# marcopesavento/Super-resolution-3D-Human-Shape-from-a-Single-Low-Resolution-Image

Hardware: AMD Instinct MI355X
Metric: occupancy queries/sec (dense 512^3 reconstruction: encoder + query sweep + 2x marching cubes) (higher is better)
Workload: dtype bf16

## Files before the change

### super-resolution-3d-human-shape-from-a-single-low-resolution-image_amd/csrc/surs_api.cpp

```cpp
#include "surs_common.h"

extern "C" int surs_abi_version(void) { return SURS_ABI_VERSION; }

extern "C" const char *surs_last_error(void) { return surs::err_buf(); }

extern "C" int surs_device_info(int *cu_count, char *arch_out) {
    int dev = 0;
    SURS_HIP_CHECK(hipGetDevice(&dev));
    hipDeviceProp_t prop;
    SURS_HIP_CHECK(hipGetDeviceProperties(&prop, dev));
    if (cu_count) *cu_count = prop.multiProcessorCount;
    if (arch_out) {
        strncpy(arch_out, prop.gcnArchName, 31);
        arch_out[31] = 0;
    }
    return 0;
}

#include <atomic>
#include <cstdlib>
#include <mutex>

namespace {
struct OptionRow {
    const char *name, *env;
    int def;
    char env_first;
    int env_value;
    const char *what;
};
const OptionRow kOptions[surs::OPT_COUNT] = {
    {"split_parts", "SURS_SPLIT", 2, 'b', 3, "operand parts of the fp32-grade GEMMs: 2 (f16 x 2) or 3 (bf16 x 3; env: bf16x3)"},
    {"grid_f32_columns", "SURS_GRID_F32", 1, 'g', 0, "0 (env: gemm): the fp32 sweep on the per-point layer kernels"},
    {"grid_kernel", "SURS_GRID_KERNEL", 0, 0, 0, "reduced-precision column kernel: 0 (default 12), 3, 10, 12"},
    {"grid_f32_kernel", "SURS_GRID_F32_KERNEL", 0, 0, 0, "fp32-grade column kernel: 0 (default 11), 5, 11"},
    {"r_parts", "SURS_R_PARTS", 1, 0, 0, "1: the bf16 sweep's R vectors from one f16 part; 0: the sweep's split"},
    {"grid_f32_passes", "SURS_GRID_F32_PASSES", 2, 0, 0, "passes of the fp32-grade column kernel per batch: 2 (lr, then hr) or 1"},
    {"bicubic_block", "SURS_BICUBIC_BLOCK", 1, 0, 0, "0: bicubic x2 with statistics one output per item (A/B; same bits)"},
    {"mc_emit_reclassify", "SURS_MC_EMIT_RECLASSIFY", 0, 0, 0, "1: marching cubes' emit pass classifies again (tests)"},
    {"point_runs_speculate", "SURS_POINT_RUNS_SPECULATE", 1, 0, 0, "0: surs_query_points_columns reads the run count before it launches"},
    {"conv_trace", "SURS_CONV_TRACE", 0, 0, 0, "diagnostic builds (-DSURS_CONV_TRACE): print the 3x3 kernel's phase stamps"},
    {"v3_trace", "SURS_V3_TRACE", 0, 0, 0, "diagnostic builds (-DSURS_V3_TRACE): print the column kernels' stamps"},
    {"conv_tall_min_wg", "SURS_CONV_TALL_MIN_WG", 256, 0, 0, "workgroups from which a stride-1 3x3 convolution takes the 8-row tile instead of 4 rows (0: never; same bits)"},
    {"conv_wide_min_wg", "SURS_CONV_WIDE_MIN_WG", 512, 0, 0, "workgroups (of 64 channels) from which such a launch takes 8 rows x 64 channels (part of the bits: another order of sums; 0: never)"},
    {"mc_ring", "SURS_MC_RING", 258, 0, 0, "planes of marching cubes' edge -> vertex-id ring = layers per chunk of a one-piece extraction + 1 (66: round 5's)"},
    {"rvec_small", "SURS_RVEC_SMALL", 1, 0, 0, "0: the affine part's GEMM of batches of <= 1024 columns on the 256 x 256-tile kernel (A/B; same bits)"},
};
std::atomic<int> g_option[surs::OPT_COUNT];
std::once_flag g_option_once;
void import_environment() {
    for (int i = 0; i < surs::OPT_COUNT; ++i) {
        const OptionRow &r = kOptions[i];
        int v = r.def;
        if (const char *e = getenv(r.env)) {
            if (r.env_first) v = (e[0] == r.env_first) ? r.env_value : r.def;
            else if (e[0]) v = atoi(e);
        }
        g_option[i].store(v, std::memory_order_relaxed);
    }
}
int find_option(const char *name) {
    if (!name) return -1;
    for (int i = 0; i < surs::OPT_COUNT; ++i)
        if (!strcmp(name, kOptions[i].name) || !strcmp(name, kOptions[i].env)) return i;
    return -1;
}
}

int surs::option(surs::Opt id) {
    std::call_once(g_option_once, import_environment);
    return g_option[id].load(std::memory_order_relaxed);
}

extern "C" int surs_set_option(const char *name, int value) {
    const int i = find_option(name);
    SURS_REQUIRE(i >= 0, "unknown option '%s' (surs_option_name(i) lists them)", name ? name : "(null)");
    std::call_once(g_option_once, import_environment);
    g_option[i].store(value, std::memory_order_relaxed);
    return 0;
}

extern "C" int surs_get_option(const char *name, int *value) {
    const int i = find_option(name);
    SURS_REQUIRE(i >= 0 && value, "unknown option '%s'", name ? name : "(null)");
    *value = surs::option((surs::Opt)i);
    return 0;
}

extern "C" const char *surs_option_name(int index) { return (index >= 0 && index < surs::OPT_COUNT) ? kOptions[index].name : nullptr; }
extern "C" const char *surs_option_help(int index) { return (index >= 0 && index < surs::OPT_COUNT) ? kOptions[index].what : nullptr; }
```

### super-resolution-3d-human-shape-from-a-single-low-resolution-image_amd/csrc/surs_common.h

```cpp
#pragma once
#include <hip/hip_runtime.h>

#include <cstdarg>
#include <cstdio>
#include <cstring>

#include "../../include/surs.h"

namespace surs {

inline char *err_buf() {
    static thread_local char buf[512] = "";
    return buf;
}

inline int fail(int code, const char *fmt, ...) {
    va_list ap;
    va_start(ap, fmt);
    vsnprintf(err_buf(), 512, fmt, ap);
    va_end(ap);
    return code;
}

#define SURS_HIP_CHECK(expr)                                                                     \
    do {                                                                                         \
        hipError_t e_ = (expr);                                                                  \
        if (e_ != hipSuccess)                                                                    \
            return surs::fail(SURS_E_HIP, "%s:%d %s -> %s", __FILE__, __LINE__, #expr, hipGetErrorString(e_)); \
    } while (0)

#define SURS_LAUNCH_CHECK() SURS_HIP_CHECK(hipGetLastError())

#define SURS_REQUIRE(cond, ...)                                   \
    do {                                                          \
        if (!(cond)) return surs::fail(SURS_E_INVALID, __VA_ARGS__); \
    } while (0)

#ifndef SURS_ABL_NO_ISA_PINS
#define SURS_ISA_PIN(v) asm volatile("" : "+v"(v))
#else
#define SURS_ISA_PIN(v) do { } while (0)
#endif

enum Opt {
    OPT_SPLIT_PARTS, OPT_GRID_F32_COLUMNS, OPT_GRID_KERNEL, OPT_GRID_F32_KERNEL, OPT_R_PARTS,
    OPT_GRID_F32_PASSES, OPT_BICUBIC_BLOCK, OPT_MC_EMIT_RECLASSIFY, OPT_POINT_RUNS_SPECULATE, OPT_CONV_TRACE,
    OPT_V3_TRACE, OPT_CONV_TALL_MIN_WG, OPT_CONV_WIDE_MIN_WG, OPT_MC_RING, OPT_RVEC_SMALL, OPT_COUNT
};
int option(Opt id);

inline hipStream_t as_stream(void *s) { return reinterpret_cast<hipStream_t>(s); }

constexpr int ceil_div(long long a, long long b) { return (int)((a + b - 1) / b); }

struct DeviceOnce {
    unsigned long long mask = 0;
    bool first() {
        int dev = 0;
        if (hipGetDevice(&dev) != hipSuccess || dev < 0 || dev >= 64) return true;
        const unsigned long long bit = 1ull << dev;
        const unsigned long long old = __atomic_fetch_or(&mask, bit, __ATOMIC_ACQ_REL);
        return !(old & bit);
    }
};
inline size_t align_up(size_t v, size_t a) { return (v + a - 1) / a * a; }

}
```

### super-resolution-3d-human-shape-from-a-single-low-resolution-image_amd/csrc/surs_gemm.inc

```
__device__ __forceinline__ bool gemm_block_tile(int mblocks, int nblocks, int &mb, int &nb) {
    const unsigned total = (unsigned)mblocks * (unsigned)nblocks, per = gridDim.x >> 3;
    const unsigned logical = (blockIdx.x & 7u) * per + (blockIdx.x >> 3);
    mb = (int)(logical % (unsigned)mblocks);
    nb = (int)(logical / (unsigned)mblocks);
    return logical < total;
}

static inline unsigned gemm_grid(int mblocks, long long nblocks) {
    const long long total = (long long)mblocks * nblocks;
    return (unsigned)(((total + 7) / 8) * 8);
}

struct SplitSeg {
    const unsigned short *base;
    long long part;
    int ktiles;
};

constexpr int G3_STAGES = 3;
constexpr int g3_stage_bytes(int bm, int np_ = 3) { return np_ * ((bm / 32) + 8) * 1024; }
constexpr int g3_lds_bytes(int bm, int np_ = 3) { return G3_STAGES * g3_stage_bytes(bm, np_); }

template <int NP> struct SplitKind;
template <> struct SplitKind<1> {
// ... 163 lines not shown
        for (int kt = 0; kt < ktiles; ++kt) {
            step_barrier(kt);
            phase1(kt);
            phase2(kt);
        }
    } else {
        step_barrier(0);
        phase1(0);
        for (int kt = 1; kt < ktiles; ++kt) {
            step_barrier(kt);
            phase2(kt - 1);
            phase1(kt);
        }
        phase2(ktiles - 1);
    }

#undef G3_RD
#undef G3_WAIT4
#undef G3_WAIT2
#pragma unroll
    for (int i = 0; i < TI; ++i)
#pragma unroll
        for (int j = 0; j < 2; ++j) {
            const long long n = n0 + wn * 64 + j * 32 + li;
            const int mrow = m0 + wm * (TI * 32) + i * 32;
            if constexpr (OUT == G3_F32_T) {
                const long long nb0 = n0 + wn * 64 + j * 32 + 4 * kh;
                const float bm = bias[mrow + li];
#pragma unroll
                for (int g = 0; g < 4; ++g)
#pragma unroll
                    for (int r = 0; r < 4; ++r) Y[(nb0 + 8 * g + r) * ldy + mrow + li] = acc[i][j][4 * g + r] + bm;
                continue;
            }
            float v[16];
#pragma unroll
            for (int g = 0; g < 4; ++g)
#pragma unroll
                for (int r = 0; r < 4; ++r) {
                    float t = acc[i][j][4 * g + r] + bias[mrow + 8 * g + 4 * kh + r];
                    v[4 * g + r] = t > 0.0f ? t : 0.01f * t;
                }
            if constexpr (OUT == G3_F32) {
#pragma unroll
                for (int g = 0; g < 4; ++g)
#pragma unroll
                    for (int r = 0; r < 4; ++r) Y[(long long)(mrow + 8 * g + 4 * kh + r) * ldy + n] = v[4 * g + r];
            } else
#pragma unroll
            for (int q = 0; q < 2; ++q) {
                unsigned e[NP][2], o[NP][2];
#pragma unroll
                for (int d = 0; d < 2; ++d) {
                    unsigned short x0[NP], x1[NP], y0[NP], y1[NP];
                    SK::split(v[8 * q + 2 * d], x0);
                    SK::split(v[8 * q + 2 * d + 1], x1);
                    SK::split(v[8 * q + 4 + 2 * d], y0);
                    SK::split(v[8 * q + 4 + 2 * d + 1], y1);
#pragma unroll
                    for (int p = 0; p < NP; ++p) {
                        e[p][d] = (unsigned)x0[p] | ((unsigned)x1[p] << 16);
                        o[p][d] = (unsigned)y0[p] | ((unsigned)y1[p] << 16);
                    }
                }
                unsigned short *dst = Ys + ((long long)((mrow >> 4) + q) * np + n) * 16 + kh * 8;
#pragma unroll
                for (int p = 0; p < NP; ++p) {
                    const auto t0 = __builtin_amdgcn_permlane32_swap(e[p][0], o[p][0], false, false);
                    const auto t1 = __builtin_amdgcn_permlane32_swap(e[p][1], o[p][1], false, false);
                    u32x4 w = {t0[0], t1[0], t0[1], t1[1]};
                    *reinterpret_cast<u32x4 *>(dst + p * ys_part) = w;
                }
            }
        }
}



struct RvecSmallArgs {
    const unsigned short *w[2];
    const unsigned short *g[2];
    long long g_part[2];
    long long npm[2];
    float *r[2];
    int wgs0;
};
template <int NP>
__global__ __launch_bounds__(256) void rvec_small_kernel(RvecSmallArgs a) {
    typedef SplitKind<NP> SK;
    typedef typename SK::vec8 vec8;
    constexpr int KT = D1 / 16, PF = 4;
    static_assert(KT % PF == 0, "k-steps in rounds of the prefetch depth");
    const int tid = threadIdx.x, lane = tid & 63, wave = tid >> 6, kh = lane >> 5, li = lane & 31;
    const int m = (int)blockIdx.x >= a.wgs0 ? 1 : 0;
    const int wg = m ? (int)blockIdx.x - a.wgs0 : (int)blockIdx.x;
    const long long npm = a.npm[m];
    const long long n0 = (long long)(wg >> 2) * 64;
    const int m0 = (wg & 3) * 128 + wave * 32;
    const size_t w_part = (size_t)D1 * D2;
    const unsigned short *wp = a.w[m] + (size_t)(m0 / 32) * 512 + lane * 8;
    const unsigned short *xp = a.g[m] + ((size_t)n0 + li) * 16 + kh * 8;
    const long long g_part = a.g_part[m];
    f32x16 acc[2];
#pragma unroll
    for (int j = 0; j < 2; ++j)
#pragma unroll
        for (int q = 0; q < 16; ++q) acc[j][q] = 0.0f;
    vec8 wf[PF][NP], xf[PF][2][NP];
    auto fetch = [&](int kt, int s) {
#pragma unroll
        for (int p = 0; p < NP; ++p) {
            wf[s][p] = *reinterpret_cast<const vec8 *>(wp + (size_t)kt * D2 * 16 + p * w_part);
#pragma unroll
            for (int j = 0; j < 2; ++j) xf[s][j][p] = *reinterpret_cast<const vec8 *>(xp + ((size_t)kt * npm + 32 * j) * 16 + p * g_part);
        }
    };
#pragma unroll
    for (int s = 0; s < PF; ++s) fetch(s, s);
    for (int k0 = 0; k0 < KT; k0 += PF) {
#pragma unroll
        for (int s = 0; s < PF; ++s) {
            vec8 w_[NP], x_[2][NP];
#pragma unroll
            for (int p = 0; p < NP; ++p) {
                w_[p] = wf[s][p];
                x_[0][p] = xf[s][0][p];
                x_[1][p] = xf[s][1][p];
            }
            if (k0 + PF + s < KT) fetch(k0 + PF + s, s);
#pragma unroll
            for (int t = 0; t < NP; ++t)
#pragma unroll
                for (int j = 0; j < 2; ++j) acc[j] = SK::mfma(x_[j][t], w_[NP - 1 - t], acc[j]);
            if (NP == 3) {
#pragma unroll
                for (int j = 0; j < 2; ++j) acc[j] = SK::mfma(x_[j][0], w_[1], acc[j]);
#pragma unroll
                for (int j = 0; j < 2; ++j) acc[j] = SK::mfma(x_[j][1], w_[0], acc[j]);
            }
            if (NP >= 2) {
#pragma unroll
                for (int j = 0; j < 2; ++j) acc[j] = SK::mfma(x_[j][0], w_[0], acc[j]);
            }
        }
    }
    float *out = a.r[m];
#pragma unroll
    for (int j = 0; j < 2; ++j)
#pragma unroll
        for (int gq = 0; gq < 4; ++gq)
#pragma unroll
            for (int r = 0; r < 4; ++r) out[(n0 + 32 * j + 4 * kh + 8 * gq + r) * D2 + m0 + li] = acc[j][4 * gq + r] + 0.0f;
}
```

### super-resolution-3d-human-shape-from-a-single-low-resolution-image_amd/csrc/surs_query.hip

```cpp
#include <hip/hip_runtime.h>

#include <cstdlib>
#include <map>
#include <mutex>
#include <type_traits>
#include <utility>
#include <vector>

#include "surs_common.h"
#include "surs_mlp_generic.h"
#include "surs_mlp_layout.h"

namespace surs {

typedef float f32x16 __attribute__((ext_vector_type(16)));
typedef float f32x4 __attribute__((ext_vector_type(4)));
typedef unsigned u32x4 __attribute__((ext_vector_type(4)));
typedef unsigned u32x2 __attribute__((ext_vector_type(2)));
typedef float f32x2 __attribute__((ext_vector_type(2)));

struct PointSource {
    int mode;
    const float *pts;
    const long long *idx;
// ... 190 lines not shown
                                                       float *__restrict__ pred, float *__restrict__ logit,
                                                       float *__restrict__ p_slot, unsigned short *__restrict__ Fs,
                                                       long long fs_part) {
    const long long t = (long long)blockIdx.x * 256 + threadIdx.x;
    if (t >= n) return;
    float acc = w4[D4 + C0PAD];
    for (int k = 0; k < D4; ++k) acc = fmaf(w4[k], Y3[(long long)k * ld + t], acc);
    for (int k = 0; k < C_G + 2; ++k) acc = fmaf(w4[D4 + k], F[(long long)k * ld + t], acc);
    const float p = mask[t] * (1.0f / (1.0f + expf(-acc)));
    pred[t] = p;
    if (logit) logit[t] = acc;
    if (p_slot) p_slot[t] = p;
    if (Fs) {
        unsigned short parts[NP];
        SplitKind<NP>::split(p, parts);
        unsigned short *dst = Fs + ((long long)(C_G / 16) * ld + t) * 16 + 1;
#pragma unroll
        for (int k = 0; k < NP; ++k) dst[k * fs_part] = parts[k];
    }
}

template <int NP>
__global__ __launch_bounds__(256) void patch_plr_kernel(const float *__restrict__ p_lr, long long ld, long long n, float *__restrict__ p_slot,
                                                        unsigned short *__restrict__ Fs, long long fs_part) {
    const long long t = (long long)blockIdx.x * 256 + threadIdx.x;
    if (t >= n) return;
    const float p = p_lr[t];
    p_slot[t] = p;
    if (Fs) {
        unsigned short parts[NP];
        SplitKind<NP>::split(p, parts);
        unsigned short *dst = Fs + ((long long)(C_G / 16) * ld + t) * 16 + 1;
#pragma unroll
        for (int k = 0; k < NP; ++k) dst[k * fs_part] = parts[k];
    }
}

__global__ __launch_bounds__(256) void mean_views_kernel(const float *__restrict__ in, long long view_stride, int nviews,
                                                         long long count, float inv, float *__restrict__ out) {
    const long long t = (long long)blockIdx.x * 256 + threadIdx.x;
    if (t >= count) return;
    float acc = in[t];
    for (int v = 1; v < nviews; ++v) acc += in[(long long)v * view_stride + t];
    out[t] = acc * inv;
}

template <int NP>
__global__ __launch_bounds__(256) void split_rows_kernel(const float *__restrict__ X, long long ld, int ktiles,
                                                         unsigned short *__restrict__ Xs, long long part) {
    const long long n = (long long)blockIdx.x * 256 + threadIdx.x;
    const int kt = blockIdx.y;
    if (n >= ld) return;
#pragma unroll
    for (int half = 0; half < 2; ++half) {
        u16x8_t q[NP];
#pragma unroll
        for (int j = 0; j < 8; ++j) {
            unsigned short parts[NP];
            SplitKind<NP>::split(X[(long long)(16 * kt + 8 * half + j) * ld + n], parts);
#pragma unroll
            for (int k = 0; k < NP; ++k) q[k][j] = parts[k];
        }
        unsigned short *dst = Xs + ((long long)kt * ld + n) * 16 + half * 8;
#pragma unroll
        for (int k = 0; k < NP; ++k) *reinterpret_cast<u16x8_t *>(dst + k * part) = q[k];
    }
}

template <int NP>
__global__ __launch_bounds__(256) void mlp_last_views_kernel(const float *__restrict__ w4, const float *__restrict__ Y3,
                                                             const float *__restrict__ Fm, long long ld, long long n,
                                                             int nviews, const float *__restrict__ mask ,
                                                             float *__restrict__ pred , float *__restrict__ logit,
                                                             float *__restrict__ p_slot ,
                                                             long long f_view_stride,
                                                             unsigned short *__restrict__ Fs ,
                                                             long long fs_part) {
    const long long t = (long long)blockIdx.x * 256 + threadIdx.x;
    if (t >= n) return;
    float acc = w4[D4 + C0PAD];
    for (int k = 0; k < D4; ++k) acc = fmaf(w4[k], Y3[(long long)k * ld + t], acc);
    for (int k = 0; k < C_G + 2; ++k) acc = fmaf(w4[D4 + k], Fm[(long long)k * ld + t], acc);
    const float y = 1.0f / (1.0f + expf(-acc));
    if (logit) logit[t] = acc;
    for (int v = 0; v < nviews; ++v) {
        const float p = mask[(long long)v * ld + t] * y;
        pred[(long long)v * n + t] = p;
        if (p_slot) p_slot[(long long)v * f_view_stride + t] = p;
        if (Fs) {
            unsigned short parts[NP];
            SplitKind<NP>::split(p, parts);
            unsigned short *dst = Fs + (long long)v * NP * fs_part + ((long long)(C_G / 16) * ld + t) * 16 + 1;
#pragma unroll
            for (int k = 0; k < NP; ++k) dst[k * fs_part] = parts[k];
        }
    }
}

struct Fp32Workspace {
    float *F, *Y3, *mask;
    unsigned short *Fs, *Y0s, *Y1s, *Y2s;
    long long np;
};

static size_t fp32_ws_bytes(long long np) {
    return (size_t)np * ((C0PAD + D4 + 1) * sizeof(float) + (size_t)(C0PAD + D1 + D2 + D3) * 6) + 4096;
}

static Fp32Workspace carve_fp32(void *ws, long long np) {
    Fp32Workspace w;
    float *p = (float *)ws;
    w.np = np;
    w.F = p; p += (size_t)C0PAD * np;
    w.Y3 = p; p += (size_t)D4 * np;
    w.mask = p; p += np;
    unsigned short *q = (unsigned short *)p;
    w.Fs = q; q += (size_t)3 * C0PAD * np;
    w.Y0s = q; q += (size_t)3 * D1 * np;
    w.Y1s = q; q += (size_t)3 * D2 * np;
    w.Y2s = q;
    return w;
}

static int g_split_override = 0;
static thread_local int t_split_call = 0;
static int split_parts() {
    const int v = option(OPT_SPLIT_PARTS) == 3 ? 3 : 2;
    return t_split_call > 1 ? t_split_call : (g_split_override ? g_split_override : v);
}

template <int NP, int... More, class F> static void with_parts(int parts, F &&f) {
    if constexpr (sizeof...(More) == 0) f(std::integral_constant<int, NP>());
    else if (parts == NP) f(std::integral_constant<int, NP>());
    else with_parts<More...>(parts, f);
}

static int g3_set_attributes() {
    static DeviceOnce attr;
    if (attr.first()) {
        SURS_HIP_CHECK(hipFuncSetAttribute((const void *)gemm_x3g_kernel<8, 256, G3_SPLIT, 2>, hipFuncAttributeMaxDynamicSharedMemorySize, g3_lds_bytes(256, 2)));
        SURS_HIP_CHECK(hipFuncSetAttribute((const void *)gemm_x3g_kernel<8, 256, G3_F32, 2>, hipFuncAttributeMaxDynamicSharedMemorySize, g3_lds_bytes(256, 2)));
        SURS_HIP_CHECK(hipFuncSetAttribute((const void *)gemm_x3g_kernel<8, 128, G3_F32, 2>, hipFuncAttributeMaxDynamicSharedMemorySize, g3_lds_bytes(128, 2)));
        SURS_HIP_CHECK(hipFuncSetAttribute((const void *)gemm_x3g_kernel<8, 128, G3_F32_T, 2>, hipFuncAttributeMaxDynamicSharedMemorySize, g3_lds_bytes(128, 2)));
        SURS_HIP_CHECK(hipFuncSetAttribute((const void *)gemm_x3g_kernel<8, 256, G3_SPLIT>, hipFuncAttributeMaxDynamicSharedMemorySize, g3_lds_bytes(256)));
        SURS_HIP_CHECK(hipFuncSetAttribute((const void *)gemm_x3g_kernel<8, 256, G3_F32>, hipFuncAttributeMaxDynamicSharedMemorySize, g3_lds_bytes(256)));
        SURS_HIP_CHECK(hipFuncSetAttribute((const void *)gemm_x3g_kernel<8, 128, G3_F32>, hipFuncAttributeMaxDynamicSharedMemorySize, g3_lds_bytes(128)));
        SURS_HIP_CHECK(hipFuncSetAttribute((const void *)gemm_x3g_kernel<8, 128, G3_F32_T>, hipFuncAttributeMaxDynamicSharedMemorySize, g3_lds_bytes(128)));
        SURS_HIP_CHECK(hipFuncSetAttribute((const void *)gemm_x3g_kernel<8, 256, G3_F32_T, 2>, hipFuncAttributeMaxDynamicSharedMemorySize, g3_lds_bytes(256, 2)));
        SURS_HIP_CHECK(hipFuncSetAttribute((const void *)gemm_x3g_kernel<8, 256, G3_F32_T>, hipFuncAttributeMaxDynamicSharedMemorySize, g3_lds_bytes(256)));
        SURS_HIP_CHECK(hipFuncSetAttribute((const void *)gemm_x3g_kernel<8, 256, G3_F32_T, 1>, hipFuncAttributeMaxDynamicSharedMemorySize, g3_lds_bytes(256, 1)));
        SURS_HIP_CHECK(hipFuncSetAttribute((const void *)gemm_x3g_kernel<8, 256, G3_SPLIT, 1>, hipFuncAttributeMaxDynamicSharedMemorySize, g3_lds_bytes(256, 1)));
        SURS_HIP_CHECK(hipFuncSetAttribute((const void *)gemm_x3g_kernel<8, 256, G3_F32, 1>, hipFuncAttributeMaxDynamicSharedMemorySize, g3_lds_bytes(256, 1)));
        SURS_HIP_CHECK(hipFuncSetAttribute((const void *)gemm_x3g_kernel<8, 128, G3_F32, 1>, hipFuncAttributeMaxDynamicSharedMemorySize, g3_lds_bytes(128, 1)));
    }
    return 0;
}

static int launch_layer(hipStream_t st, int parts, int out, const void *W, int M, SplitSeg s1, SplitSeg s2, long long np, long long n,
                        const float *bias, float *Y, unsigned short *Ys) {
    SURS_REQUIRE(parts >= 1 && parts <= 3, "layer kernel: 1, 2 or 3 operand parts");
    SURS_REQUIRE(np % 256 == 0 && n % 256 == 0 && n <= np, "the layer kernel needs 256-point tiles");
    SURS_REQUIRE(M % 256 == 0 || (out != G3_SPLIT && M % 128 == 0), "layer kernel rows: a multiple of 256 (of 128 for an fp32 output)");
    SURS_REQUIRE(M % 256 == 0 || out != G3_F32_T || parts > 1, "no one-part layer kernel for a transposed output of 128-row tiles");
    int rc = g3_set_attributes();
    if (rc) return rc;
    const int K = 16 * (s1.ktiles + s2.ktiles), nb = (int)(n / 256);
    const long long ldy = out == G3_F32_T ? M : np;
    with_parts<1, 2, 3>(parts, [&](auto NP) {
        auto go = [&](auto BM, auto OUT) {
            hipLaunchKernelGGL((gemm_x3g_kernel<8, BM, OUT, NP>), dim3(gemm_grid(M / BM, nb)), dim3(512), g3_lds_bytes(BM, NP), st,
                               (const unsigned short *)W, M, K, s1, s2, np, bias, Y, ldy, Ys, (long long)M * np, nb);
        };
        using C256 = std::integral_constant<int, 256>;
        using C128 = std::integral_constant<int, 128>;
        if (out == G3_SPLIT) go(C256(), std::integral_constant<int, G3_SPLIT>());
        else if (out == G3_F32) {
            if (M % 256 == 0) go(C256(), std::integral_constant<int, G3_F32>());
            else go(C128(), std::integral_constant<int, G3_F32>());
        } else if (M % 256 == 0) go(C256(), std::integral_constant<int, G3_F32_T>());
        else if constexpr (NP > 1) go(C128(), std::integral_constant<int, G3_F32_T>());
    });
    SURS_LAUNCH_CHECK();
    return 0;
}

static int run_points_fp32(hipStream_t st, const PointSource &src, long long n, const float *feat_lr, int hl, int wl,
                           const float *feat_hr, int hh, int wh, const char *blob, const MlpBlobHeader &h,
                           const Fp32Workspace &w, float *pred_hr, float *pred_lr, float *logit_hr, float *logit_lr,
                           int parts = 0, const float *p_lr_in = nullptr, bool lr_only = false) {
    const long long np = w.np;
    if (parts == 0) parts = t_split_call == 1 ? 1 : split_parts();
    const long long fs_part = (long long)C0PAD * np;
    with_parts<1, 2, 3>(parts, [&](auto NP) {
        hipLaunchKernelGGL(gather_kernel<NP>, dim3((unsigned)ceil_div(n, 64)), dim3(256), 0, st, src, n, feat_lr, hl, wl, feat_hr,
                           hh, wh, w.F, np, w.mask, (float *)nullptr, w.Fs, fs_part);
    });
    SURS_LAUNCH_CHECK();
    if (p_lr_in) {
        with_parts<1, 2, 3>(parts, [&](auto NP) {
            hipLaunchKernelGGL(patch_plr_kernel<NP>, dim3((unsigned)ceil_div(n, 256)), dim3(256), 0, st, p_lr_in, np, n,
                               w.F + (size_t)(C_G + 1) * np, w.Fs, fs_part);
        });
        SURS_LAUNCH_CHECK();
    }
    const SplitSeg none = {nullptr, 0, 0}, f = {w.Fs, fs_part, C0PAD / 16}, y0 = {w.Y0s, (long long)D1 * np, D1 / 16},
                   y1 = {w.Y1s, (long long)D2 * np, D2 / 16}, y2 = {w.Y2s, (long long)D3 * np, D3 / 16};
    for (int m = p_lr_in ? 1 : 0; m < (lr_only ? 1 : 2); ++m) {
        auto W = [&](int l) { return (const void *)(blob + (parts <= 2 ? h.wt2[m][l] : h.wt3[m][l])); };
        auto BI = [&](int l) { return (const float *)(blob + h.bias[m][l]); };
        int rc;
        if ((rc = launch_layer(st, parts, G3_SPLIT, W(0), D1, f, none, np, np, BI(0), nullptr, w.Y0s))) return rc;
        if ((rc = launch_layer(st, parts, G3_SPLIT, W(1), D2, y0, none, np, np, BI(1), nullptr, w.Y1s))) return rc;
        if ((rc = launch_layer(st, parts, G3_SPLIT, W(2), D3, y1, f, np, np, BI(2), nullptr, w.Y2s))) return rc;
        if ((rc = launch_layer(st, parts, G3_F32, W(3), D4, y2, f, np, np, BI(3), w.Y3, nullptr))) return rc;
        with_parts<1, 2, 3>(parts, [&](auto NP) {
            hipLaunchKernelGGL(mlp_last_kernel<NP>, dim3((unsigned)ceil_div(n, 256)), dim3(256), 0, st,
                               (const float *)(blob + h.w4[m]), w.Y3, w.F, np, n, w.mask, m == 0 ? pred_lr : pred_hr,
                               m == 0 ? logit_lr : logit_hr, m == 0 ? w.F + (size_t)(C_G + 1) * np : (float *)nullptr,
                               m == 0 ? w.Fs : (unsigned short *)nullptr, fs_part);
        });
        SURS_LAUNCH_CHECK();
    }
    return 0;
}

template <int DT> struct HalfT;
template <> struct HalfT<SURS_BF16> {
    typedef __bf16 elem;
    typedef __bf16 vec8 __attribute__((ext_vector_type(8)));
    typedef __bf16 vec2 __attribute__((ext_vector_type(2)));
    static __device__ __forceinline__ f32x16 mfma(vec8 a, vec8 b, f32x16 c) {
        return __builtin_amdgcn_mfma_f32_32x32x16_bf16(a, b, c, 0, 0, 0);
    }
};
template <> struct HalfT<SURS_F16> {
    typedef _Float16 elem;
    typedef _Float16 vec8 __attribute__((ext_vector_type(8)));
    typedef _Float16 vec2 __attribute__((ext_vector_type(2)));
    static __device__ __forceinline__ f32x16 mfma(vec8 a, vec8 b, f32x16 c) {
        return __builtin_amdgcn_mfma_f32_32x32x16_f16(a, b, c, 0, 0, 0);
    }
};

struct GridArgs {
    const float *cc;
    const float *colmask;
    const float *zvec;
    const char *core;
    const char *corex;
    const char *b1frag;
    const char *w1t;
    const char *w1tx;
    const float *rvec_lr, *rvec_hr;
    long long rld_lr, rld_hr;
    float zmid;
    unsigned *colctr;
    int phase;
    unsigned long long *kstat;
    float b1_inv_scale;
    float *vol_hr, *vol_lr;
    int ncols, rz;
    int zstride;
    const int *kcount;
    const unsigned short *klist;
    const int *colstart;
    const float *zpts;
    unsigned *ovf_count;
    int *ovf_list;
    char *aimg;
    const int *tile_list;
    const unsigned *tile_count;
    double z0, dz;
    float c22, c23;
    float zmul, zdiv;
};

__device__ __forceinline__ float lrelu_max(float x, float y) { return __builtin_elementwise_maximum(x, y); }
__device__ __forceinline__ float lrelu01(float x) { return lrelu_max(x, 0.01f * x); }

__device__ __forceinline__ unsigned opaque(unsigned v) {
    asm volatile("" : "+v"(v));
    return v;
}
__device__ __forceinline__ unsigned fresh_lane() {
    unsigned v;
    asm volatile("v_mbcnt_lo_u32_b32 %0, -1, 0\n\tv_mbcnt_hi_u32_b32 %0, -1, %0" : "=v"(v));
    return v;
}

#include "surs_grid_v3.inc"
#include "surs_grid_v5.inc"
#include "surs_grid_restated.inc"
#include "surs_grid_v10.inc"
#include "surs_grid_v12.inc"
#include "surs_grid_v11.inc"

template <int NP>
__global__ __launch_bounds__(256) void colsum_prepare_kernel(const float *__restrict__ cc, const float *__restrict__ zvec, int ncp,
                                                             float zmid, unsigned short *__restrict__ g_lr, long long part_lr,
                                                             unsigned short *__restrict__ g_hr, long long part_hr) {
    typedef SplitKind<NP> SK;
    __shared__ __attribute__((aligned(16))) unsigned stage[64][20][8];
    const int tid = threadIdx.x, lane = tid & 63, wave = tid >> 6;
    const int col0 = blockIdx.x * 4, col = col0 + wave;
    const int c16 = lane;
    const float *row = cc + (size_t)col * CC_PAD + 16 * c16;
// ... 429 lines not shown
        const float Z = c23 + c22 * zw;
        return Z * zmul / zdiv;
    };
    unsigned nl = 0, nh = 0;
    for (int k0 = 0; k0 < rz; k0 += tile) {
        const float e0 = zf_of(k0), e1 = zf_of(k0 + tile - 1);
        const float zlo = fminf(e0, e1), zhi = fmaxf(e0, e1);
#pragma unroll
        for (int i = 0; i < 4; ++i) {
            {
                const float xm = fmaf(zmid, zl[i], al[i]);
                const float t0 = zl[i] * zlo, t1 = zl[i] * zhi;
                const float mn = al[i] + fminf(t0, t1), mx = al[i] + fmaxf(t0, t1);
                nl += ((xm > 0.0f) ? (mn > 0.0f) : (mx <= 0.0f)) ? 0u : 1u;
            }
            {
                const float xm = fmaf(0.5f, ph[i], fmaf(zmid, zh[i], ah[i]));
                const float t0 = zh[i] * zlo, t1 = zh[i] * zhi;
                const float mn = ah[i] + fminf(t0, t1) + fminf(0.0f, ph[i]), mx = ah[i] + fmaxf(t0, t1) + fmaxf(0.0f, ph[i]);
                nh += ((xm > 0.0f) ? (mn > 0.0f) : (mx <= 0.0f)) ? 0u : 1u;
            }
        }
    }
#pragma unroll
    for (int d = 32; d >= 1; d >>= 1) {
        nl += __shfl_xor(nl, d);
        nh += __shfl_xor(nh, d);
    }
    if ((tid & 63) == 0) {
        atomicAdd(out, (unsigned long long)nl);
        atomicAdd(out + 1, (unsigned long long)nh);
    }
}

static int query_grid_impl(int i0, int i1, int ry, int rz, const double *mat, const float *calib, float zmul,
                           float zdiv, const float *feat_lr, int hl, int wl, const float *feat_hr, int hh, int wh,
                           const void *mlp_blob, int dtype, void *workspace, size_t workspace_bytes, float *vol_hr,
                           float *vol_lr, int kernel_call, void *stream);

extern "C" int surs_query_grid_opt(int i0, int i1, int ry, int rz, const double *mat, const float *calib, float zmul,
                                   float zdiv, const float *feat_lr, int hl, int wl, const float *feat_hr, int hh, int wh,
                                   const void *mlp_blob, int dtype, void *workspace, size_t workspace_bytes, float *vol_hr,
                                   float *vol_lr, const SursGridOptions *opt, void *stream) {
    int kernel = 0, parts = 0;
    if (opt) {
        kernel = opt->kernel;
        parts = opt->operand_parts;
        SURS_REQUIRE(grid_kernel_known(kernel), "SursGridOptions.kernel: 0, 3, 10, 12 (reduced precision), 5, 11 (fp32-grade)");
        SURS_REQUIRE(parts == 0 || parts == 2 || parts == 3, "SursGridOptions.operand_parts: 0, 2 or 3");
    }
    const int saved = t_split_call;
    if (parts) t_split_call = parts;
    const int rc = query_grid_impl(i0, i1, ry, rz, mat, calib, zmul, zdiv, feat_lr, hl, wl, feat_hr, hh, wh, mlp_blob, dtype, workspace,
                                   workspace_bytes, vol_hr, vol_lr, kernel, stream);
    t_split_call = saved;
    return rc;
}

extern "C" int surs_query_grid(int i0, int i1, int ry, int rz, const double *mat, const float *calib, float zmul,
                               float zdiv, const float *feat_lr, int hl, int wl, const float *feat_hr, int hh, int wh,
                               const void *mlp_blob, int dtype, void *workspace, size_t workspace_bytes, float *vol_hr,
                               float *vol_lr, void *stream) {
    return query_grid_impl(i0, i1, ry, rz, mat, calib, zmul, zdiv, feat_lr, hl, wl, feat_hr, hh, wh, mlp_blob, dtype, workspace,
                           workspace_bytes, vol_hr, vol_lr, 0, stream);
}

namespace {
struct ColumnSweep {
    hipStream_t st;
    const char *blob;
    MlpBlobHeader h;
    int dtype;
    int kver, kver32;
    bool restated;
    const float *feat_lr; int hl, wl;
    const float *feat_hr; int hh, wh;
    const double *mat; const float *calib; float zmul, zdiv;
    void *workspace;
    int cus;
    int kmid;
    const int *run_colstart = nullptr;
    const float *run_z = nullptr;
    const int *run_tiles = nullptr;
    const unsigned *run_ntiles = nullptr;
    long long run_ntiles_host = 0;
};
}

static void resolve_column_kernels(int kernel_call, int &kver, int &kver32) {
    const int ve = option(OPT_GRID_KERNEL), ve32 = option(OPT_GRID_F32_KERNEL);
    const int kver_env = (ve == 3 || ve == 10 || ve == 12) ? ve : SURS_DEFAULT_GRID_KERNEL;
    const int kver32_env = (ve32 == 5 || ve32 == 11) ? ve32 : SURS_DEFAULT_GRID_F32_KERNEL;
    const auto is32 = [](int v) { return v == 5 || v == 11; };
    kver = kver_env;
    kver32 = kver32_env;
    if (g_grid_kernel_override) (is32(g_grid_kernel_override) ? kver32 : kver) = g_grid_kernel_override;
    if (kernel_call) (is32(kernel_call) ? kver32 : kver) = kernel_call;
}

static int device_cus() {
    int dev = 0;
    hipDeviceProp_t prop;
    if (hipGetDevice(&dev) == hipSuccess && hipGetDeviceProperties(&prop, dev) == hipSuccess) return prop.multiProcessorCount;
    return 256;
}

static int run_column_batch(const ColumnSweep &cs, const PointSource &src, long long nc, int items, int zstride,
                            const int *kcount, const unsigned short *klist, float *vol_hr, float *vol_lr, bool trace_this) {
    hipStream_t st = cs.st;
    const char *blob = cs.blob;
    const MlpBlobHeader &h = cs.h;
    const int dtype = cs.dtype, kver = cs.kver, kver32 = cs.kver32;
    const bool restated = cs.restated;
    const double *mat = cs.mat;
    const float *calib = cs.calib;
    void *workspace = cs.workspace;
    float *F = (float *)workspace;
    float *CC = F + (size_t)C0PAD * COL_BATCH;
    float *cmask = CC + (size_t)CC_PAD * COL_BATCH;
    int rc = 0;
    const long long ncp = (long long)ceil_div(nc, 256) * 256;
    const int parts = split_parts();
    if ((rc = column_constants(st, src, nc, ncp, cs.feat_lr, cs.hl, cs.wl, cs.feat_hr, cs.hh, cs.wh, blob, h, F, CC, cmask))) return rc;
    GridArgs a;
    a.cc = CC;
    a.colmask = cmask;
    a.zvec = (const float *)(blob + h.zvec);
    a.core = blob + h.core;
    a.corex = blob + h.corex;
    a.b1frag = blob + h.b1frag;
    a.b1_inv_scale = 1.0f / (dtype == SURS_F16 ? B1FRAG_SCALE_F16 : B1FRAG_SCALE_BF16);
    a.w1t = blob + h.w1t;
    a.w1tx = blob + h.w1tx;
    a.rvec_lr = a.rvec_hr = nullptr;
    a.rld_lr = a.rld_hr = 0;
    a.colctr = nullptr;
    a.phase = 0;
    a.zmid = 0.0f;
    a.zstride = zstride;
    a.kcount = kcount;
    a.klist = klist;
    a.ovf_count = nullptr;
    a.ovf_list = nullptr;
    a.aimg = nullptr;
    a.tile_list = cs.run_tiles;
    a.tile_count = cs.run_ntiles;
    a.colstart = cs.run_colstart;
    a.zpts = cs.run_z;
    if (restated) {
        char *v7 = (char *)workspace + col_base_bytes(COL_BATCH);
        unsigned short *g_lr = (unsigned short *)v7, *g_hr = g_lr + (size_t)COL_BATCH * 2 * D1 * 3;
        float *r_lr = (float *)(v7 + col_v7_image_bytes(COL_BATCH)), *r_hr = r_lr + (size_t)COL_BATCH * 2 * D2;
        float *zero_bias = r_hr + (size_t)COL_BATCH * 3 * D2;
        SURS_HIP_CHECK(hipMemsetAsync(zero_bias, 0, D2 * 4 + 256, st));
        a.colctr = (unsigned *)(zero_bias + D2);
        {
            const float zw = cs.run_z ? 0.0f : (float)(mat[10] * (double)cs.kmid + mat[11]);
            a.zmid = (calib[11] + calib[10] * zw) * cs.zmul / cs.zdiv;
        }
        const long long part_lr = 2LL * ncp * D1, part_hr = 3LL * ncp * D1;
        const dim3 pg((unsigned)(ncp / 4));
        const int r_parts_env = option(OPT_R_PARTS);
        const int rparts = (dtype == SURS_BF16 && r_parts_env == 1) ? 1 : parts;
        with_parts<1, 2, 3>(rparts, [&](auto NP) {
            hipLaunchKernelGGL(colsum_prepare_kernel<NP>, pg, dim3(256), 0, st, CC, (const float *)(blob + h.zvec), (int)ncp, a.zmid,
                               g_lr, part_lr, g_hr, part_hr);
        });
        SURS_LAUNCH_CHECK();
        if (ncp <= 1024 && option(OPT_RVEC_SMALL)) {
            RvecSmallArgs ra;
            for (int m = 0; m < 2; ++m) {
                const int nvec = m ? 3 : 2;
                ra.w[m] = (const unsigned short *)(blob + (rparts == 3 ? h.wt3[m][1] : h.wt2[m][1]));
                ra.g[m] = m ? g_hr : g_lr;
                ra.g_part[m] = m ? part_hr : part_lr;
                ra.npm[m] = (long long)nvec * ncp;
                ra.r[m] = m ? r_hr : r_lr;
            }
            ra.wgs0 = (int)(ra.npm[0] / 64) * 4;
            const unsigned wgs = (unsigned)(ra.wgs0 + (ra.npm[1] / 64) * 4);
            with_parts<1, 2, 3>(rparts, [&](auto NP) { hipLaunchKernelGGL(rvec_small_kernel<NP>, dim3(wgs), dim3(256), 0, st, ra); });
            SURS_LAUNCH_CHECK();
        } else {
            const SplitSeg none = {nullptr, 0, 0};
            for (int m = 0; m < 2; ++m) {
                const long long npm = (m ? 3LL : 2LL) * ncp;
                const SplitSeg g = {m ? g_hr : g_lr, m ? part_hr : part_lr, D1 / 16};
                if ((rc = launch_layer(st, rparts, G3_F32_T, blob + (rparts == 3 ? h.wt3[m][1] : h.wt2[m][1]), D2, g, none, npm, npm,
                                       zero_bias, m ? r_hr : r_lr, nullptr)))
                    return rc;
            }
        }
        a.rvec_lr = r_lr;
        a.rvec_hr = r_hr;
        a.rld_lr = a.rld_hr = 0;
    }
    a.vol_hr = vol_hr;
    a.vol_lr = vol_lr;
    a.ncols = (int)nc;
    a.rz = items;
    a.z0 = mat ? mat[11] : 0.0;
    a.dz = mat ? mat[10] : 0.0;
    a.c22 = calib[10];
    a.c23 = calib[11];
    a.zmul = cs.zmul;
    a.zdiv = cs.zdiv;
    const long long nwork = cs.run_tiles ? cs.run_ntiles_host : nc;
    const unsigned grid = (unsigned)((nwork < cs.cus) ? nwork : cs.cus);
    hipEvent_t e0 = nullptr, e1 = nullptr;
    bool prof;
    a.kstat = nullptr;
    {
        std::lock_guard<std::mutex> lock(g_prof.mu);
        prof = g_prof.on && !kcount;
        if (prof && restated) {
            int dev = 0;
            SURS_HIP_CHECK(hipGetDevice(&dev));
            unsigned long long *&ctr = g_prof.kstat[dev];
            if (!ctr) {
                SURS_HIP_CHECK(hipMalloc((void **)&ctr, sizeof(unsigned long long)));
                SURS_HIP_CHECK(hipMemset(ctr, 0, sizeof(unsigned long long)));
            }
            a.kstat = ctr;
            g_prof.tiles += 2.0 * (double)nc * (dtype == SURS_F32 ? (items + 63) / 64 : (items + 127) / 128);
        }
    }
    if (prof) {
        SURS_HIP_CHECK(hipEventCreate(&e0));
        SURS_HIP_CHECK(hipEventCreate(&e1));
        SURS_HIP_CHECK(hipEventRecord(e0, st));
    }
    if (dtype == SURS_F32) {
        if (kver32 == 11) {
            const int passes_env = option(OPT_GRID_F32_PASSES);
            const bool two = passes_env == 2 && items % 64 == 0 && !cs.run_tiles;
            for (int ph = two ? 1 : 0; ph <= (two ? 2 : 0); ++ph) {
                a.phase = ph;
                hipLaunchKernelGGL(grid_mlp_kernel_v11, dim3(grid), dim3(V11_THREADS), GRID11_LDS_BYTES, st, a);
            }
        } else
            hipLaunchKernelGGL(grid_mlp_kernel_v5, dim3(grid), dim3(256), GRID5_LDS_BYTES, st, a);
    } else if (kver == 12) {
#ifdef SURS_V12_ONE_WG
        const unsigned grid12 = (unsigned)((nc < cs.cus) ? nc : cs.cus);
#else
        const unsigned grid12 = (unsigned)((nc < 2 * cs.cus) ? nc : 2 * cs.cus);
#endif
        a.ovf_count = a.colctr + 1;
        a.ovf_list = (int *)((char *)workspace + col_base_bytes(COL_BATCH));
        const size_t ovf_room = ((size_t)nc * ((items + 127) / 128) * 2 * sizeof(int) + 4095) / 4096 * 4096;
        SURS_REQUIRE(ovf_room + (size_t)grid12 * V12_AIMG_BYTES <= col_v7_image_bytes(COL_BATCH),
                     "kernel v12's overflow list and fragment images do not fit the g-scaled split image");
        a.aimg = (char *)a.ovf_list + ovf_room;
        const int lds12 = GRID12_LDS_BYTES;
        if (dtype == SURS_BF16)
            hipLaunchKernelGGL(grid_mlp_kernel_v12<SURS_BF16>, dim3(grid12), dim3(V12_THREADS), lds12, st, a);
        else
            hipLaunchKernelGGL(grid_mlp_kernel_v12<SURS_F16>, dim3(grid12), dim3(V12_THREADS), lds12, st, a);
        SURS_LAUNCH_CHECK();
        GridArgs b = a;
        b.tile_list = a.ovf_list;
        b.tile_count = a.ovf_count;
        b.colctr = a.colctr + 2;
        if (dtype == SURS_BF16)
            hipLaunchKernelGGL(grid_mlp_kernel_v10<SURS_BF16>, dim3(grid), dim3(V10_THREADS), GRID10_LDS_BYTES, st, b);
        else
            hipLaunchKernelGGL(grid_mlp_kernel_v10<SURS_F16>, dim3(grid), dim3(V10_THREADS), GRID10_LDS_BYTES, st, b);
    } else if (kver == 10) {
        if (dtype == SURS_BF16)
            hipLaunchKernelGGL(grid_mlp_kernel_v10<SURS_BF16>, dim3(grid), dim3(V10_THREADS), GRID10_LDS_BYTES, st, a);
        else
            hipLaunchKernelGGL(grid_mlp_kernel_v10<SURS_F16>, dim3(grid), dim3(V10_THREADS), GRID10_LDS_BYTES, st, a);
    } else {
        if (dtype == SURS_BF16)
            hipLaunchKernelGGL(grid_mlp_kernel_v3<SURS_BF16>, dim3(grid), dim3(256), GRID3_LDS_BYTES, st, a);
        else
            hipLaunchKernelGGL(grid_mlp_kernel_v3<SURS_F16>, dim3(grid), dim3(256), GRID3_LDS_BYTES, st, a);
    }
    SURS_LAUNCH_CHECK();
#ifdef SURS_V12_HIST
    if (kver == 12 && dtype != SURS_F32) {
        static unsigned long long *hist = nullptr;
        if (!hist) {
            SURS_HIP_CHECK(hipMalloc((void **)&hist, 65 * 8));
            SURS_HIP_CHECK(hipMemset(hist, 0, 65 * 8));
            SURS_HIP_CHECK(hipMemcpyToSymbol(HIP_SYMBOL(g_v12_hist), &hist, sizeof(hist)));
            static unsigned long long *h2 = hist;
            atexit([] {
                unsigned long long v[65];
                if (hipMemcpy(v, h2, sizeof(v), hipMemcpyDeviceToHost) != hipSuccess) return;
                unsigned long long tot = 0;
                for (int i = 0; i < 65; ++i) tot += v[i];
                fprintf(stderr, "v12 tiles by residual k-steps (total %llu):", tot);
                for (int i = 0; i < 65; ++i) if (v[i]) fprintf(stderr, " %d:%.4f", i, (double)v[i] / (double)tot);
                fprintf(stderr, "\n");
            });
        }
    }
#endif
#ifdef SURS_V3_TRACE
    if (trace_this && option(OPT_V3_TRACE)) {
        unsigned long long t[64];
        SURS_HIP_CHECK(hipStreamSynchronize(st));
        SURS_HIP_CHECK(hipMemcpyFromSymbol(t, HIP_SYMBOL(g_v3_trace), sizeof(t)));
        for (int m = 0; m < 2; ++m) {
            fprintf(stderr, "v3 trace MLP %d:", m);
            for (int i = 1; i < 10; ++i) fprintf(stderr, " %llu", t[16 * m + i] - t[16 * m + i - 1]);
            fprintf(stderr, "  total %llu\n", t[16 * m + 9] - t[16 * m]);
            if (restated) {
                fprintf(stderr, "   v7 layer 1 (since start): init issued %llu, list %llu, chunk 0: gathered %llu, residuals %llu, barrier %llu, mfma+barrier %llu; listed %llu\n",
                        t[16 * m + 10] - t[16 * m], t[16 * m + 1] - t[16 * m], t[16 * m + 11] - t[16 * m], t[16 * m + 12] - t[16 * m],
                        t[16 * m + 13] - t[16 * m], t[16 * m + 14] - t[16 * m], t[48 + m]);
            }
        }
        fprintf(stderr, "v3 trace between MLPs: %llu\n", t[16] - t[9]);
        if (kver == 12 && dtype != SURS_F32) {
            unsigned long long acc[2][16];
            SURS_HIP_CHECK(hipMemcpyFromSymbol(acc, HIP_SYMBOL(g_v12_acc), sizeof(acc)));
            for (int m = 0; m < 2; ++m) {
                const double n = (double)(acc[m][0] ? acc[m][0] : 1);
                double tot = 0;
                fprintf(stderr, "v12 mean cycles per item, MLP %d (%llu items, %.2f residual k-steps): ", m, acc[m][0], (double)acc[m][15] / n);
// ... 653 lines not shown
```

Before: 1.154 billion.

## Fuse g-scaled image formation into a single R-vector GEMM kernel for large batches

For bf16 sweeps with one-part R vectors and batches over 1024 columns, a new kernel computes the leaky-gate scaling of the column sums, splits the values to half precision into LDS, and runs the MFMA GEMM for both the lr and hr phases in one launch. This replaces the separate colsum_prepare kernel, the global g-image round trip, the two GEMM launches, and most of the zero-bias memset. The cost is a more complex double-buffered kernel with heavy register use that recomputes gating per output-row tile. It is gated by a new option that is on by default.

```diff
diff --git a/super-resolution-3d-human-shape-from-a-single-low-resolution-image_amd/csrc/surs_api.cpp b/super-resolution-3d-human-shape-from-a-single-low-resolution-image_amd/csrc/surs_api.cpp
--- a/super-resolution-3d-human-shape-from-a-single-low-resolution-image_amd/csrc/surs_api.cpp
+++ b/super-resolution-3d-human-shape-from-a-single-low-resolution-image_amd/csrc/surs_api.cpp
@@ -45,6 +45,7 @@
     {"conv_wide_min_wg", "SURS_CONV_WIDE_MIN_WG", 512, 0, 0, "workgroups (of 64 channels) from which such a launch takes 8 rows x 64 channels (part of the bits: another order of sums; 0: never)"},
     {"mc_ring", "SURS_MC_RING", 258, 0, 0, "planes of marching cubes' edge -> vertex-id ring = layers per chunk of a one-piece extraction + 1 (66: round 5's)"},
     {"rvec_small", "SURS_RVEC_SMALL", 1, 0, 0, "0: the affine part's GEMM of batches of <= 1024 columns on the 256 x 256-tile kernel (A/B; same bits)"},
+    {"r_fused", "SURS_R_FUSED", 1, 0, 0, "0: the bf16 sweep's R vectors of batches of > 1024 columns from the g-scaled image and two GEMM launches (A/B; same bits)"},
 };
 std::atomic<int> g_option[surs::OPT_COUNT];
 std::once_flag g_option_once;
diff --git a/super-resolution-3d-human-shape-from-a-single-low-resolution-image_amd/csrc/surs_common.h b/super-resolution-3d-human-shape-from-a-single-low-resolution-image_amd/csrc/surs_common.h
--- a/super-resolution-3d-human-shape-from-a-single-low-resolution-image_amd/csrc/surs_common.h
+++ b/super-resolution-3d-human-shape-from-a-single-low-resolution-image_amd/csrc/surs_common.h
@@ -45,7 +45,7 @@
 enum Opt {
     OPT_SPLIT_PARTS, OPT_GRID_F32_COLUMNS, OPT_GRID_KERNEL, OPT_GRID_F32_KERNEL, OPT_R_PARTS,
     OPT_GRID_F32_PASSES, OPT_BICUBIC_BLOCK, OPT_MC_EMIT_RECLASSIFY, OPT_POINT_RUNS_SPECULATE, OPT_CONV_TRACE,
-    OPT_V3_TRACE, OPT_CONV_TALL_MIN_WG, OPT_CONV_WIDE_MIN_WG, OPT_MC_RING, OPT_RVEC_SMALL, OPT_COUNT
+    OPT_V3_TRACE, OPT_CONV_TALL_MIN_WG, OPT_CONV_WIDE_MIN_WG, OPT_MC_RING, OPT_RVEC_SMALL, OPT_R_FUSED, OPT_COUNT
 };
 int option(Opt id);
 
diff --git a/super-resolution-3d-human-shape-from-a-single-low-resolution-image_amd/csrc/surs_gemm.inc b/super-resolution-3d-human-shape-from-a-single-low-resolution-image_amd/csrc/surs_gemm.inc
--- a/super-resolution-3d-human-shape-from-a-single-low-resolution-image_amd/csrc/surs_gemm.inc
+++ b/super-resolution-3d-human-shape-from-a-single-low-resolution-image_amd/csrc/surs_gemm.inc
@@ -339,3 +339,150 @@
 #pragma unroll
             for (int r = 0; r < 4; ++r) out[(n0 + 32 * j + 4 * kh + 8 * gq + r) * D2 + m0 + li] = acc[j][4 * gq + r] + 0.0f;
 }
+
+struct RvecFusedArgs {
+    const float *cc;
+    const float *zvec;
+    const unsigned short *w[2];
+    float *r[2];
+    float zmid;
+    int tiles;
+};
+constexpr int RVF_COLS = 64, RVF_ROWS = 256, RVF_THREADS = 512;
+constexpr int RVF_KS = 8;
+constexpr int RVF_PIECE = 1040, RVF_HALF = 528;
+constexpr int RVF_STAGE_BYTES = RVF_KS * 6 * RVF_PIECE;
+constexpr int RVF_Z_BYTES = 2 * D1 * 4;
+constexpr int RVF_LDS_BYTES = 2 * RVF_STAGE_BYTES + RVF_Z_BYTES;
+
+template <int M>
+__device__ __forceinline__ void rvec_fused_phase(const RvecFusedArgs &a, unsigned char *smem, int col0, int m0) {
+    typedef SplitKind<1> SK;
+    typedef SK::vec8 vec8;
+    constexpr int NV = M ? 3 : 2, NT = 2 * NV;
+    constexpr int KS = RVF_KS, STEPS = D1 / (16 * KS), KT = D1 / 16, PF = RVF_KS, NQ = RVF_COLS / 16, PS = RVF_PIECE;
+    static_assert(KS * NT * PS <= RVF_STAGE_BYTES && STEPS % 2 == 0 && KS == PF && KS >= NQ && KS % 2 == 0, "stage size; steps in pairs");
+    const int tid = threadIdx.x, lane = tid & 63, kh = lane >> 5, li = lane & 31;
+    const int fc = tid >> 5, fq = tid & 31;
+    const float *crow = a.cc + (size_t)(col0 + fc) * CC_PAD + (M ? CC_A0_HR : CC_A0_LR) + 4 * fq;
+    const float zmid = a.zmid;
+    float *zs = reinterpret_cast<float *>(smem + 2 * RVF_STAGE_BYTES);
+    {
+        const int v = tid >> 8, c = 4 * (tid & 255);
+        if (M || v == 0)
+            *reinterpret_cast<f32x4 *>(zs + v * D1 + c) =
+                *reinterpret_cast<const f32x4 *>(a.zvec + (v ? ZV_W0P_HR : (M ? ZV_W0Z_HR : ZV_W0Z_LR)) + c);
+    }
+    const unsigned wbase = (unsigned)(((fq >> 2) * NT * PS) + (((fq & 3) >> 1) * RVF_HALF) + (fq & 1) * 8);
+    auto load = [&](int s, int q) {
+        return *reinterpret_cast<const f32x4 *>(crow + (size_t)(16 * q) * CC_PAD + 16 * KS * s);
+    };
+    auto form = [&](int q, const f32x4 a0, const f32x4 wz, const f32x4 wp, unsigned char *stage) {
+        unsigned short hw[NV][4];
+#pragma unroll
+        for (int e = 0; e < 4; ++e) {
+            float g, val[3];
+            if constexpr (M) {
+                g = fmaf(0.5f, wp[e], fmaf(zmid, wz[e], a0[e])) > 0.0f ? 1.0f : 0.01f;
+                val[2] = g * wp[e];
+            } else {
+                g = fmaf(zmid, wz[e], a0[e]) > 0.0f ? 1.0f : 0.01f;
+                val[2] = 0.0f;
+            }
+            val[0] = g * a0[e];
+            val[1] = g * wz[e];
+#pragma unroll
+            for (int v = 0; v < NV; ++v) {
+                unsigned short p[1];
+                SK::split(val[v], p);
+                hw[v][e] = p[0];
+            }
+        }
+#pragma unroll
+        for (int v = 0; v < NV; ++v) {
+            const int p = (fc + 16 * q) * NV + v;
+            *reinterpret_cast<u32x2 *>(stage + wbase + (unsigned)((p >> 5) * PS + (p & 31) * 16)) =
+                u32x2{(unsigned)hw[v][0] | ((unsigned)hw[v][1] << 16), (unsigned)hw[v][2] | ((unsigned)hw[v][3] << 16)};
+        }
+    };
+    auto zload = [&](int s, f32x4 &wz, f32x4 &wp) {
+        wz = *reinterpret_cast<const f32x4 *>(zs + 16 * KS * s + 4 * fq);
+        wp = wz;
+        if constexpr (M) wp = *reinterpret_cast<const f32x4 *>(zs + D1 + 16 * KS * s + 4 * fq);
+    };
+    const unsigned short *wp_ = a.w[M] + (size_t)(m0 / 32) * 512 + lane * 8;
+    auto wload = [&](int kt) { return *reinterpret_cast<const vec8 *>(wp_ + (size_t)kt * D2 * 16); };
+    f32x16 acc[NT];
+#pragma unroll
+    for (int j = 0; j < NT; ++j)
+#pragma unroll
+        for (int q = 0; q < 16; ++q) acc[j][q] = 0.0f;
+    vec8 wf[PF];
+#pragma unroll
+    for (int k = 0; k < PF; ++k) wf[k] = wload(k);
+    f32x4 ring[NQ];
+#pragma unroll
+    for (int q = 0; q < NQ; ++q) ring[q] = load(0, q);
+    __syncthreads();
+    {
+        f32x4 wz, wp;
+        zload(0, wz, wp);
+#pragma unroll
+        for (int q = 0; q < NQ; ++q) {
+            form(q, ring[q], wz, wp, smem);
+            ring[q] = load(1, q);
+        }
+    }
+    __syncthreads();
+    const unsigned char *rd = smem + kh * RVF_HALF + li * 16;
+    vec8 x[2][NT];
+#pragma unroll
+    for (int j = 0; j < NT; ++j) x[0][j] = *reinterpret_cast<const vec8 *>(rd + j * PS);
+#pragma unroll 1
+    for (int s2 = 0; s2 < STEPS; s2 += 2) {
+#pragma unroll
+        for (int u = 0; u < 2; ++u) {
+            const int s = s2 + u;
+            const int sf = s + 1 < STEPS ? s + 1 : STEPS - 1, sl = s + 2 < STEPS ? s + 2 : STEPS - 1;
+#pragma unroll
+            for (int t = 0; t < KS; ++t) {
+                const int kt = KS * s + t;
+                if (t + 1 < KS) {
+#pragma unroll
+                    for (int j = 0; j < NT; ++j)
+                        x[(t + 1) & 1][j] = *reinterpret_cast<const vec8 *>(rd + u * RVF_STAGE_BYTES + ((t + 1) * NT + j) * PS);
+                }
+                __builtin_amdgcn_sched_barrier(0);
+                const vec8 w = wf[t];
+#pragma unroll
+                for (int j = 0; j < NT; ++j) acc[j] = SK::mfma(x[t & 1][j], w, acc[j]);
+                if (t < NQ) {
+                    f32x4 wz, wp;
+                    zload(sf, wz, wp);
+                    form(t, ring[t], wz, wp, smem + (u ^ 1) * RVF_STAGE_BYTES);
+                    ring[t] = load(sl, t);
+                }
+                wf[t] = wload(kt + PF < KT ? kt + PF : KT - 1);
+            }
+            __syncthreads();
+#pragma unroll
+            for (int j = 0; j < NT; ++j) x[0][j] = *reinterpret_cast<const vec8 *>(rd + (u ^ 1) * RVF_STAGE_BYTES + j * PS);
+        }
+    }
+    float *out = a.r[M] + (size_t)col0 * NV * D2 + m0 + li;
+#pragma unroll
+    for (int j = 0; j < NT; ++j)
+#pragma unroll
+        for (int gq = 0; gq < 4; ++gq)
+#pragma unroll
+            for (int r = 0; r < 4; ++r) out[(size_t)(32 * j + 4 * kh + 8 * gq + r) * D2] = acc[j][4 * gq + r] + 0.0f;
+}
+
+__global__ __launch_bounds__(RVF_THREADS) void rvec_fused_kernel(RvecFusedArgs a) {
+    extern __shared__ __attribute__((aligned(16))) unsigned char rvf_smem[];
+    int mb, nb;
+    if (!gemm_block_tile(D2 / RVF_ROWS, a.tiles, mb, nb)) return;
+    const int col0 = nb * RVF_COLS, m0 = mb * RVF_ROWS + (int)(threadIdx.x >> 6) * 32;
+    rvec_fused_phase<0>(a, rvf_smem, col0, m0);
+    rvec_fused_phase<1>(a, rvf_smem, col0, m0);
+}
diff --git a/super-resolution-3d-human-shape-from-a-single-low-resolution-image_amd/csrc/surs_query.hip b/super-resolution-3d-human-shape-from-a-single-low-resolution-image_amd/csrc/surs_query.hip
--- a/super-resolution-3d-human-shape-from-a-single-low-resolution-image_amd/csrc/surs_query.hip
+++ b/super-resolution-3d-human-shape-from-a-single-low-resolution-image_amd/csrc/surs_query.hip
@@ -366,6 +366,7 @@
         SURS_HIP_CHECK(hipFuncSetAttribute((const void *)gemm_x3g_kernel<8, 256, G3_SPLIT, 1>, hipFuncAttributeMaxDynamicSharedMemorySize, g3_lds_bytes(256, 1)));
         SURS_HIP_CHECK(hipFuncSetAttribute((const void *)gemm_x3g_kernel<8, 256, G3_F32, 1>, hipFuncAttributeMaxDynamicSharedMemorySize, g3_lds_bytes(256, 1)));
         SURS_HIP_CHECK(hipFuncSetAttribute((const void *)gemm_x3g_kernel<8, 128, G3_F32, 1>, hipFuncAttributeMaxDynamicSharedMemorySize, g3_lds_bytes(128, 1)));
+        SURS_HIP_CHECK(hipFuncSetAttribute((const void *)rvec_fused_kernel, hipFuncAttributeMaxDynamicSharedMemorySize, RVF_LDS_BYTES));
     }
     return 0;
 }
@@ -1101,7 +1102,6 @@
         unsigned short *g_lr = (unsigned short *)v7, *g_hr = g_lr + (size_t)COL_BATCH * 2 * D1 * 3;
         float *r_lr = (float *)(v7 + col_v7_image_bytes(COL_BATCH)), *r_hr = r_lr + (size_t)COL_BATCH * 2 * D2;
         float *zero_bias = r_hr + (size_t)COL_BATCH * 3 * D2;
-        SURS_HIP_CHECK(hipMemsetAsync(zero_bias, 0, D2 * 4 + 256, st));
         a.colctr = (unsigned *)(zero_bias + D2);
         {
             const float zw = cs.run_z ? 0.0f : (float)(mat[10] * (double)cs.kmid + mat[11]);
@@ -1111,12 +1111,30 @@
         const dim3 pg((unsigned)(ncp / 4));
         const int r_parts_env = option(OPT_R_PARTS);
         const int rparts = (dtype == SURS_BF16 && r_parts_env == 1) ? 1 : parts;
-        with_parts<1, 2, 3>(rparts, [&](auto NP) {
-            hipLaunchKernelGGL(colsum_prepare_kernel<NP>, pg, dim3(256), 0, st, CC, (const float *)(blob + h.zvec), (int)ncp, a.zmid,
-                               g_lr, part_lr, g_hr, part_hr);
-        });
-        SURS_LAUNCH_CHECK();
-        if (ncp <= 1024 && option(OPT_RVEC_SMALL)) {
+        const bool fused = rparts == 1 && ncp > 1024 && option(OPT_R_FUSED);
+        if (fused) SURS_HIP_CHECK(hipMemsetAsync(a.colctr, 0, 256, st));
+        else SURS_HIP_CHECK(hipMemsetAsync(zero_bias, 0, D2 * 4 + 256, st));
+        if (!fused) {
+            with_parts<1, 2, 3>(rparts, [&](auto NP) {
+                hipLaunchKernelGGL(colsum_prepare_kernel<NP>, pg, dim3(256), 0, st, CC, (const float *)(blob + h.zvec), (int)ncp, a.zmid,
+                                   g_lr, part_lr, g_hr, part_hr);
+            });
+            SURS_LAUNCH_CHECK();
+        }
+        if (fused) {
+            RvecFusedArgs fa;
+            fa.cc = CC;
+            fa.zvec = (const float *)(blob + h.zvec);
+            fa.zmid = a.zmid;
+            fa.tiles = (int)(ncp / RVF_COLS);
+            for (int m = 0; m < 2; ++m) {
+                fa.w[m] = (const unsigned short *)(blob + h.wt2[m][1]);
+                fa.r[m] = m ? r_hr : r_lr;
+            }
+            if ((rc = g3_set_attributes())) return rc;
+            hipLaunchKernelGGL(rvec_fused_kernel, dim3(gemm_grid(D2 / RVF_ROWS, fa.tiles)), dim3(RVF_THREADS), RVF_LDS_BYTES, st, fa);
+            SURS_LAUNCH_CHECK();
+        } else if (ncp <= 1024 && option(OPT_RVEC_SMALL)) {
             RvecSmallArgs ra;
             for (int m = 0; m < 2; ++m) {
                 const int nvec = m ? 3 : 2;
```

New measurement: 1.170 billion, median of 6. +1.4%, better.
